# jgdumas/plinopt

Hardware: AMD Instinct MI355X
Metric: candidate SLPs/sec (higher is better)
Workload: dtype u32

## Files before the change

plinopt_amd/csrc/plo_cse_big.hip:

```cpp
#include <hip/hip_runtime.h>
#include <stdint.h>
#include <type_traits>

namespace plo {

#ifndef PLO_BIG_THREADS
#define PLO_BIG_THREADS 512
#endif
#define PLO_BIG_SELCAP 512u
#define PLO_GVB 16u
#define PLO_GVMASK 0xFFFFull
#define PLO_GEMPTY 0xFFFFFFFFFFFF0000ull

struct BigPlan {
    uint32_t m, n, nnz, p, NCmax, hbits, rb, bb, unit, maxf0, M0, multcap, dmcap, hlcap, scr_stride, aggbits, mers, agg_cb, agg_dual, selcap, prune;
    uint64_t mu;
    uint32_t nv, vt_lds;
    uint32_t mode, nr;
    const uint16_t *rtid, *invid;
    const uint32_t *rval;
    const uint32_t *rs, *ent0, *tptr, *trows, *ucount0, *hist0;
    const uint2 *vt;
    const uint32_t *invtab;
    const uint64_t *tab0;
// ... 263 lines not shown
        const uint32_t s1 = (s + 1u) & mask;
        const uint64_t v0 = __hip_atomic_load(&agg[s], __ATOMIC_RELAXED, __HIP_MEMORY_SCOPE_WORKGROUP), v1 = __hip_atomic_load(&agg[s1], __ATOMIC_RELAXED, __HIP_MEMORY_SCOPE_WORKGROUP);
        const bool hit0 = (v0 >> acb) == key, emp0 = v0 == EMPTY, first = hit0 || emp0;
        const bool hit = hit0 || (!emp0 && (v1 >> acb) == key), emp = emp0 || (!hit && v1 == EMPTY);
        const uint32_t t = first ? s : s1;
        if (hit) { wg_add((unsigned long long *)&agg[t], 1ull); done = true; break; }
        if (emp) {
            const uint64_t old = wg_cas((unsigned long long *)&agg[t], (unsigned long long)EMPTY, (unsigned long long)((key << acb) | 1ull));
            if (old == EMPTY) { claimed = t; done = true; break; }
            continue;
        }
        s = (s + 2u) & mask; pr += 2u;
    }
    const unsigned long long cm = __builtin_amdgcn_ballot_w64(claimed != 0xFFFFFFFFu);
    if (cm) {
        const uint32_t lane = threadIdx.x & 63u, leader = (uint32_t)__builtin_ctzll(cm);
        uint32_t base = 0;
        if (lane == leader) base = wg_add(aggn, (uint32_t)__builtin_popcountll(cm));
        base = (uint32_t)__builtin_amdgcn_readlane((int)base, (int)leader);
        if (claimed != 0xFFFFFFFFu) {
            const uint32_t idx = base + (uint32_t)__builtin_popcountll(cm & ((1ull << lane) - 1ull));
            if (idx < listcap) agglist[idx] = (uint16_t)claimed;
        }
    }
    return done;
}

#define PLO_RIDB 10u
#define PLO_RSTRIDE 32u
struct BigTabs { const uint2 *vts; const uint16_t *rtid; const uint32_t *rval; const uint16_t *invid; uint16_t *list; uint32_t *bloom; };
__device__ __forceinline__ bool agg_add_rid(uint32_t *aggk, uint32_t *aggc32, uint32_t aggbits, uint32_t key, uint32_t *aggn, uint16_t *agglist, uint32_t listcap) {
    const uint32_t mask = (1u << aggbits) - 1u;
    uint32_t s = (key * 0x9E3779B1u) >> (32u - aggbits);
    uint32_t claimed = 0xFFFFFFFFu; bool done = false;
    for (uint32_t pr = 0; pr < PLO_AGG_PROBES;) {
        const uint32_t s1 = (s + 1u) & mask;
        const uint32_t k0 = __hip_atomic_load(&aggk[s], __ATOMIC_RELAXED, __HIP_MEMORY_SCOPE_WORKGROUP), k1 = __hip_atomic_load(&aggk[s1], __ATOMIC_RELAXED, __HIP_MEMORY_SCOPE_WORKGROUP);
        const bool hit0 = k0 == key, emp0 = k0 == 0xFFFFFFFFu, first = hit0 || emp0;
        const bool hit = hit0 || (!emp0 && k1 == key), emp = emp0 || (!hit && k1 == 0xFFFFFFFFu);
        const uint32_t t = first ? s : s1;
        if (hit) { wg_add(&aggc32[t >> 1], 1u << ((t & 1u) << 4)); done = true; break; }
        if (emp) {
            const uint32_t old = wg_cas(&aggk[t], 0xFFFFFFFFu, key);
            if (old == 0xFFFFFFFFu || old == key) { if (old != key) claimed = t; wg_add(&aggc32[t >> 1], 1u << ((t & 1u) << 4)); done = true; break; }
            continue;
        }
        s = (s + 2u) & mask; pr += 2u;
    }
    const unsigned long long cm = __builtin_amdgcn_ballot_w64(claimed != 0xFFFFFFFFu);
    if (cm) {
        const uint32_t lane = threadIdx.x & 63u, leader = (uint32_t)__builtin_ctzll(cm);
        uint32_t base = 0;
        if (lane == leader) base = wg_add(aggn, (uint32_t)__builtin_popcountll(cm));
        base = (uint32_t)__builtin_amdgcn_readlane((int)base, (int)leader);
        if (claimed != 0xFFFFFFFFu) {
            const uint32_t idx = base + (uint32_t)__builtin_popcountll(cm & ((1ull << lane) - 1ull));
            if (idx < listcap) agglist[idx] = (uint16_t)claimed;
        }
    }
    return done;
}

__device__ __forceinline__ bool agg_add_rid_bm(uint32_t *aggk, uint32_t *aggc32, uint32_t aggbits, uint32_t key, uint32_t hshift, uint32_t *iters = nullptr) {
    const uint32_t pmask = (1u << (aggbits - 1u)) - 1u;
    uint32_t pi = (uint32_t)__umul24(key, 0x9E3779u) >> hshift;
    for (uint32_t left = PLO_AGG_PROBES / 2u;;) {
        if (iters) ++*iters;
        const unsigned long long kk = __hip_atomic_load((unsigned long long *)aggk + pi, __ATOMIC_RELAXED, __HIP_MEMORY_SCOPE_WORKGROUP);
        const uint32_t k0 = (uint32_t)kk, k1 = (uint32_t)(kk >> 32);
        const bool first = k0 == key || k0 == 0xFFFFFFFFu;
        const uint32_t kt = first ? k0 : k1;
        bool mine = kt == key;
        const uint32_t next = !mine && kt != 0xFFFFFFFFu ? 1u : 0u;
        if (kt == 0xFFFFFFFFu) {
            const uint32_t sec = first ? 0u : 1u;
            const uint32_t old = wg_cas((uint32_t *)((unsigned long long *)aggk + pi) + sec, 0xFFFFFFFFu, key);
            mine = old == 0xFFFFFFFFu || old == key;
        }
        if (mine) wg_add(&aggc32[pi], first ? 1u : 0x10000u);
        pi = (pi + next) & pmask; left -= next;
        if (mine || left == 0u) return mine;
    }
}

#ifdef PLO_BIG_PROFILE
__device__ __forceinline__ bool agg_add_rid_first_prof(uint32_t *aggk, uint32_t *aggc32, uint32_t aggbits, uint32_t key, unsigned long long *acc) {
    const unsigned long long c0 = clock64();
    const uint32_t s = ((uint32_t)__umul24(key, 0x9E3779u) >> (32u - aggbits)) & ~1u;
    const unsigned long long kk = __hip_atomic_load((unsigned long long *)(aggk + s), __ATOMIC_RELAXED, __HIP_MEMORY_SCOPE_WORKGROUP);
    const uint32_t k0 = (uint32_t)kk, k1 = (uint32_t)(kk >> 32);
    asm volatile("s_waitcnt lgkmcnt(0)" ::: "memory"); const unsigned long long c1 = clock64();
    const bool hit0 = k0 == key, hit = hit0 || k1 == key, emp0 = k0 == 0xFFFFFFFFu, tryc = !hit && (emp0 || k1 == 0xFFFFFFFFu);
    const uint32_t sec = hit ? (hit0 ? 0u : 1u) : (emp0 ? 0u : 1u), t = s + sec;
    uint32_t old = 0u;
    if (tryc) old = wg_cas(&aggk[t], 0xFFFFFFFFu, key);
    asm volatile("s_waitcnt lgkmcnt(0)" ::: "memory"); const unsigned long long c2 = clock64();
    const bool ok = hit || (tryc && (old == 0xFFFFFFFFu || old == key));
    if (ok) wg_add(&aggc32[s >> 1], sec ? 0x10000u : 1u);
    asm volatile("s_waitcnt lgkmcnt(0)" ::: "memory"); const unsigned long long c3 = clock64();
    acc[0] += c1 - c0; acc[1] += c2 - c1; acc[2] += c3 - c2;
    return !ok;
}
#endif

#define PLO_ECOL(e_) ((e_) & 0x7FFFu)
#define PLO_EUNIT(e_) (((e_) >> 15) & 1u)
#define PLO_EVI(e_) ((e_) >> 16)
#define PLO_RW_LEN 0x3FFFu
#define PLO_RW_NEW 0x1F8000u
#define PLO_RW_VIB 22u
#define PLO_RW_VIA 27u
template <class ENT> __device__ __forceinline__ int row_find(ENT ent, uint32_t base, uint32_t L, uint32_t c) {
    uint32_t lo = 0, hi = L;
    while (lo < hi) { uint32_t mid = (lo + hi) >> 1; if (PLO_ECOL(ent[base + mid]) < c) lo = mid + 1; else hi = mid; }
    return (lo < L && PLO_ECOL(ent[base + lo]) == c) ? (int)lo : -1;
}

struct BigShared {
    uint32_t M, theta, ncols, nbadd, nbmul, nmult, naff, dmcount, hlcount, rng, errflag, sel_n, sel_over, invr, fullscans, rebuilds, steps, hlbad, acc0, acc1;
    uint32_t a, b, r, aggn, nspill, keepn; uint64_t kprime; uint64_t selkey;
    uint32_t nbisect, spilltot, listover, nwin, nsearched;
    uint32_t logn, hotn, hotbits, nforced, hotops, logtot_lo, logtot_hi;
    uint32_t derr; unsigned long long tmg[4], tmb[4]; uint32_t ngrp, nloop; uint32_t outcnt[64];
    uint32_t cblk[512];
    unsigned long long tph[8];
    unsigned long long tpg[7], tld;
#ifdef PLO_BIG_PROFILE
    unsigned long long tb1[4], tb2[4]; uint32_t nb[4], fb1, fb2, fl1, fl2;
    unsigned long long tpc[4][8];
    unsigned long long pw[16];
#endif
    uint32_t part[8];
    uint64_t sel[PLO_BIG_SELCAP];
};

#define BSYNC() __syncthreads()
#ifdef PLO_BIG_PROFILE
#define PLO_STAMP(q_) do { if (threadIdx.x == 0) { unsigned long long t_ = wall_clock64(); sh.tph[q_] += t_ - tstamp; sh.tpc[sh.M >= 256u ? 0 : sh.M >= 64u ? 1 : sh.M >= 16u ? 2 : 3][q_] += t_ - tstamp; tstamp = t_; } } while (0)
#else
#define PLO_STAMP(q_) do { if (threadIdx.x == 0) { unsigned long long t_ = wall_clock64(); sh.tph[q_] += t_ - tstamp; tstamp = t_; } } while (0)
#endif

#define PLO_DLB 13u
#define PLO_DCH 4096u
#define PLO_DBIAS 0x8000u
#define PLO_DBLOOM_WORDS 4096u
#define PLO_DMREG_WORDS 16384u
#define PLO_DPMAX 2048u
#define PLO_LEMPTY (~0ull)
static_assert(PLO_DPMAX <= 4u * PLO_BIG_THREADS && PLO_DCH % PLO_BIG_THREADS == 0u && 2u * PLO_DCH + 3u * PLO_DPMAX <= PLO_DMREG_WORDS, "merge layout");

__device__ __forceinline__ uint64_t dmix(uint64_t key) { return key * 0x9E3779B97F4A7C15ull; }
__device__ __forceinline__ uint32_t dpart(uint64_t key, uint32_t pbits) { return pbits ? (uint32_t)(dmix(key) >> (64u - pbits)) : 0u; }
__device__ __forceinline__ uint32_t dlslot(uint64_t key, uint32_t pbits, uint32_t lb) { return (uint32_t)((dmix(key) << pbits) >> (64u - lb)); }
__device__ __forceinline__ bool dbloom_test(const uint32_t *bl, uint64_t key) {
    const uint64_t g = key * 0xD6E8FEB86659FD93ull;
    const uint32_t i1 = (uint32_t)(g >> 47), i2 = (uint32_t)(g >> 30) & 0x1FFFFu, i3 = (uint32_t)(g >> 13) & 0x1FFFFu;
    const uint32_t w1 = __hip_atomic_load(&bl[i1 >> 5], __ATOMIC_RELAXED, __HIP_MEMORY_SCOPE_WORKGROUP), w2 = __hip_atomic_load(&bl[i2 >> 5], __ATOMIC_RELAXED, __HIP_MEMORY_SCOPE_WORKGROUP),
                   w3 = __hip_atomic_load(&bl[i3 >> 5], __ATOMIC_RELAXED, __HIP_MEMORY_SCOPE_WORKGROUP);
    return (((w1 >> (i1 & 31u)) & (w2 >> (i2 & 31u)) & (w3 >> (i3 & 31u))) & 1u) != 0u;
}
__device__ __forceinline__ void dbloom_set(uint32_t *bl, uint64_t key) {
    const uint64_t g = key * 0xD6E8FEB86659FD93ull;
    const uint32_t i1 = (uint32_t)(g >> 47), i2 = (uint32_t)(g >> 30) & 0x1FFFFu, i3 = (uint32_t)(g >> 13) & 0x1FFFFu;
    wg_or(&bl[i1 >> 5], 1u << (i1 & 31u)); wg_or(&bl[i2 >> 5], 1u << (i2 & 31u)); wg_or(&bl[i3 >> 5], 1u << (i3 & 31u));
}
template <class TAB> __device__ __forceinline__ uint32_t hot_slot(TAB hot, uint64_t key, uint32_t hb, uint64_t &v) {
    const uint32_t mask = (1u << hb) - 1u;
    uint32_t s = ghash(key, hb);
    for (uint32_t pr = 0; pr <= mask; ++pr) {
        v = gload64(&hot[s]);
        if ((v >> PLO_GVB) == key) return s;
        if (v == PLO_GEMPTY) return 0xFFFFFFFFu;
        s = (s + 1u) & mask;
    }
    return 0xFFFFFFFFu;
}
template <class TAB> __device__ __forceinline__ uint32_t hot_addn(TAB hot, uint64_t key, uint32_t d, uint32_t hb, uint32_t *hotn) {
    const uint32_t mask = (1u << hb) - 1u;
    uint32_t s = ghash(key, hb);
    for (uint32_t pr = 0; pr <= 2u * mask + 1u; ++pr) {
        const uint64_t v = gload64(&hot[s]);
        if ((v >> PLO_GVB) == key) { const uint64_t old = wg_add((unsigned long long *)&hot[s], (unsigned long long)d); return (uint32_t)(old & PLO_GVMASK); }
        if (v == PLO_GEMPTY) {
            const uint64_t old = wg_cas((unsigned long long *)&hot[s], (unsigned long long)v, (unsigned long long)((key << PLO_GVB) | d));
            if (old == v) { wg_add(hotn, 1u); return 0u; }
// ... 496 lines not shown
        const bool swap = gload32(&ucount[a]) < gload32(&ucount[b]);
        const uint32_t l0 = swap ? b : a, l1 = swap ? a : b;
        if (tid == 0) { sh.naff = 0; sh.aggn = 0; sh.nspill = 0; sh.keepn = 0; }
        BSYNC();
#define RL(v_, k_) ((uint32_t)__builtin_amdgcn_readlane((int)(v_), (int)(k_)))
        A32 wlst; uint32_t lc;
        {
            const A32 la = a < n ? tl + tptr[a] : ncr + ncrptr[a - n], lb = b < n ? tl + tptr[b] : ncr + ncrptr[b - n];
            const uint32_t na = gload32(&clen[a]), nb = gload32(&clen[b]);
            const bool walk_a = na <= nb;
            const A32 lst = walk_a ? la : lb; const uint32_t ln = walk_a ? na : nb;
            wlst = lst; lc = walk_a ? a : b;
            if (tid == 0) sh.nsearched += ln;
            const A32 newrows = ncr + ncrptr[lm - n];
            auto emit = [&](uint32_t i, uint32_t base, uint32_t L, uint32_t pa, uint32_t pb, uint32_t ea, uint32_t eb) -> bool {
                uint32_t inv_r;
                if constexpr (MODE == 2) {
                    if (rval[rtid[PLO_EVI(eb) * PLO_RSTRIDE + PLO_EVI(ea)]] != r) return false;
                    inv_r = rval[rtid[PLO_EVI(ea) * PLO_RSTRIDE + PLO_EVI(eb)]];
                } else {
                    const uint2 A = VT(PLO_EVI(ea)), B = VT(PLO_EVI(eb));
                    if (B.x != bmul(r, A.x, p, mu, mers)) return false;
                    inv_r = bmul(A.x, B.y, p, mu, mers);
                }
                const uint32_t idx = wg_add(&sh.naff, 1u);
#ifdef PLO_BIG_PROFILE
                atomicAdd(&sh.tb2[1], 100ull * L);
#endif
                if constexpr (MODE == 2) {
                    *(uint4 *)(aff + 4u * idx) = make_uint4(pa | (pb << 16), base, L | ((swap ? eb : ea) & PLO_RW_NEW) | (PLO_EVI(eb) << PLO_RW_VIB) | (PLO_EVI(ea) << PLO_RW_VIA), i);
                } else {
                uint32_t *rec = &aff[8u * idx];
                *(uint4 *)rec = make_uint4(i, pa | (pb << 16), base, L);
                *(uint2 *)(rec + 4) = make_uint2(ea, eb);
                }
                newrows[idx] = i;
                if (idx == 0) sh.invr = inv_r;
                len[i] = L - 1u;
                if (PLO_EUNIT(ea)) wg_sub(&ucount[a], 1u);
                if (PLO_EUNIT(eb)) wg_sub(&ucount[b], 1u);
                if (PLO_EUNIT(swap ? eb : ea)) wg_add(&ucount[lm], 1u);
                return true;
            };
            auto keep_row = [&](uint32_t i, bool has_col, bool affected) { if (has_col && !affected) keep[wg_add(&sh.keepn, 1u)] = i; };
#ifdef PLO_BIG_PROFILE
            if (tid == 0) { sh.tb2[0] += 100ull * ln; sh.tb2[2] += 100ull * (na <= nb ? nb : na); }
#endif
            for (uint32_t k = tid; k < ln; k += 2u * nth) {
                const bool two = k + nth < ln;
                const uint32_t i0 = lst[k], i1 = two ? lst[k + nth] : i0;
                const uint32_t bs0 = rs[i0], bs1 = rs[i1], L0 = len[i0], L1 = two ? len[i1] : 0u;
                uint32_t lo[4] = {0u, 0u, 0u, 0u}, hi[4] = {L0, L0, L1, L1}, ev[4] = {0xFFFFFFFFu, 0xFFFFFFFFu, 0xFFFFFFFFu, 0xFFFFFFFFu};
                for (;;) {
                    uint32_t v[4], mid[4]; bool any = false;
#pragma unroll
                    for (int q = 0; q < 4; ++q) {
                        mid[q] = (lo[q] + hi[q]) >> 1; const bool go = lo[q] < hi[q]; any |= go;
                        v[q] = go ? ent[(q < 2 ? bs0 : bs1) + mid[q]] : 0u;
                    }
                    if (!any) break;
#pragma unroll
                    for (int q = 0; q < 4; ++q)
                        if (lo[q] < hi[q]) { if (PLO_ECOL(v[q]) < ((q & 1) ? b : a)) lo[q] = mid[q] + 1u; else { hi[q] = mid[q]; ev[q] = v[q]; } }
                }
                {   const bool fa = PLO_ECOL(ev[0]) == a && lo[0] < L0, fb = PLO_ECOL(ev[1]) == b && lo[1] < L0;
                    const bool aff0 = fa && fb && emit(i0, bs0, L0, lo[0], lo[1], ev[0], ev[1]);
                    keep_row(i0, walk_a ? fa : fb, aff0); }
                if (two) { const bool fa = PLO_ECOL(ev[2]) == a && lo[2] < L1, fb = PLO_ECOL(ev[3]) == b && lo[3] < L1;
                    const bool aff1 = fa && fb && emit(i1, bs1, L1, lo[2], lo[3], ev[2], ev[3]);
                    keep_row(i1, walk_a ? fa : fb, aff1); }
            }
        }
        PLO_BIG_FENCE(); BSYNC();
        const uint32_t naff = sh.naff;
        {
            const uint32_t nk = sh.keepn;
            for (uint32_t k = tid; k < nk; k += nth) wlst[k] = keep[k];
            if (tid == 0) clen[lc] = nk;
        }
        PLO_STAMP(2);
        if (naff != M) { if (tid == 0) wg_max(&sh.errflag, (uint32_t)BERR_FREQ); BSYNC(); break; }
        {
#ifdef PLO_BIG_PROFILE
            uint32_t probe_iters = 0; unsigned long long pq[3] = {0, 0, 0}, prt = 0;
#endif
            uint32_t aggsh = 33u - aggbits; asm("" : "+v"(aggsh));
            const uint32_t agg_dual = MODE == 2 ? 0u : PW(agg_dual), logcap = DEFER ? PW(logcap) : 0u;
            auto retire_entry = [&](uint32_t e, uint32_t rw, bool above, uint2 VA, uint2 VB, bool noagg = false) {
                const uint32_t c = PLO_ECOL(e);
                uint32_t x, y, q2, ins;
                if constexpr (MODE == 2) {
                    const uint32_t vi = PLO_EVI(e), via = rw >> PLO_RW_VIA;
#ifdef PLO_BIG_PROFILE
                    const unsigned long long cr0 = clock64();
#endif
                    const uint32_t xid = rtid[((above ? vi : via) * PLO_RSTRIDE) | (above ? via : vi)];
#ifdef PLO_BIG_PROFILE
                    if constexpr (FAST) {
                        asm volatile("s_waitcnt lgkmcnt(0)" ::: "memory"); prt += clock64() - cr0;
                        const bool pend = agg_add_rid_first_prof(aggk, aggc32, aggbits, (c << PLO_RIDB) | xid, pq);
                        if (!__builtin_amdgcn_ballot_w64(pend)) return;
                        if (!pend || agg_add_rid_bm(aggk, aggc32, aggbits, (c << PLO_RIDB) | xid, aggsh, &probe_iters)) return;
                    }
#else
                    if constexpr (FAST) { if (!noagg) { if (__builtin_expect(agg_add_rid_bm(aggk, aggc32, aggbits, (c << PLO_RIDB) | xid, aggsh), 1)) return; } }
#endif
                    else if (agg_add_rid(aggk, aggc32, aggbits, (c << PLO_RIDB) | xid, &sh.aggn, agglist, listcap)) return;
                    const uint32_t vib = (rw >> PLO_RW_VIB) & 31u;
                    const uint32_t bc = rval[rtid[vib * PLO_RSTRIDE + vi]];
                    x = rval[xid]; y = rval[rtid[via * PLO_RSTRIDE + vi]];
                    q2 = c < b ? bc : rval[rtid[vi * PLO_RSTRIDE + vib]];
                    ins = l0 == a ? y : bc;
                } else {
                    const uint2 V = VT(PLO_EVI(e));
                    y = bmul(VA.x, V.y, p, mu, mers);
                    x = c < a ? y : bmul(V.x, VA.y, p, mu, mers);
                    const uint64_t cx = ((uint64_t)c << rb) | x;
                    if (agg_add(agg, aggbits, acb, agg_dual ? (cx << rb) | y : cx, (uint32_t)cx ^ ((uint32_t)(cx >> 32) * 0x85EBCA6Bu), &sh.aggn, agglist, listcap)) return;
                    q2 = c < b ? bmul(VB.x, V.y, p, mu, mers) : bmul(V.x, VB.y, p, mu, mers);
                    ins = bmul(l0 == a ? VA.x : VB.x, V.y, p, mu, mers);
                }
#ifdef PLO_BIG_PROFILE
                wg_add(&sh.fb1, 1u);
#endif
                const uint64_t k1 = c < a ? BKEY(c, a, x) : BKEY(a, c, x);
                const uint64_t k2 = c < b ? BKEY(c, b, q2) : BKEY(b, c, q2);
                if constexpr (DEFER) {
                    for (int w_ = 0; w_ < 2; ++w_) {
                        const uint64_t kk = w_ ? k2 : k1; const uint32_t fc = w_ ? (c < b ? c : b) : (c < a ? c : a);
                        bool done = false;
                        if (dbloom_test(bloom, kk)) {
                            uint64_t v; const uint32_t sl = hot_slot(tab, kk, hbits, v);
                            if (sl != 0xFFFFFFFFu) {
                                const uint32_t o = (uint32_t)(wg_add((unsigned long long *)&tab[sl], ~0ull) & PLO_GVMASK);
                                if (o) { wg_sub(&hist[o], 1u); if (o > 1u) wg_add(&hist[o - 1u], 1u); if (o == M) { wg_sub(&cntM[fc], 1u); wg_sub(&sh.cblk[fc >> 6], 1u); } }
                                else wg_max(&sh.errflag, (uint32_t)BERR_TABLE);
                                done = true;
                            }
                        }
                        if (!done) { const uint32_t li = wg_add(&sh.logn, 1u); if (li < logcap) dlog[li] = PLO_DREC(kk, 1u, false); else wg_max(&sh.errflag, (uint32_t)BERR_TABLE); }
                    }
                    const uint32_t idx = wg_add(&sh.nspill, 1u);
                    if (idx < spillcap) spill[idx] = BKEY(c, lm, ins); else wg_max(&sh.errflag, (uint32_t)BERR_TABLE);
                    return;
                }
                const uint32_t o1 = gtab_dec(tab, k1, hbits);
                if (o1) {
                    wg_sub(&hist[o1], 1u); if (o1 > 1u) wg_add(&hist[o1 - 1u], 1u);
                    if (o1 == M) { wg_sub(&cntM[c < a ? c : a], 1u); wg_sub(&sh.cblk[(c < a ? c : a) >> 6], 1u); }
                }
                const uint32_t o2 = gtab_dec(tab, k2, hbits);
                if (o2) {
                    wg_sub(&hist[o2], 1u); if (o2 > 1u) wg_add(&hist[o2 - 1u], 1u);
                    if (o2 == M) { wg_sub(&cntM[c < b ? c : b], 1u); wg_sub(&sh.cblk[(c < b ? c : b) >> 6], 1u); }
                }
                const uint32_t idx = wg_add(&sh.nspill, 1u);
                if (idx < spillcap) spill[idx] = BKEY(c, lm, ins); else wg_max(&sh.errflag, (uint32_t)BERR_TABLE);
            };
            const uint32_t nrw = naff > wave ? (naff - wave + nwaves - 1u) / nwaves : 0u;
#ifdef PLO_BIG_PROFILE
            unsigned long long pw0 = 0, pw1 = 0, pw2 = 0, ptr = 0, pit = 0, pact = 0, tl_ = clock64(); const unsigned long long ts_ = tl_;
#endif
            if constexpr (FAST) {
            uint64_t *fm = sh.sel + 256u + 32u * wave;
            const uint32_t FW = PW(fwin);
            const uint32_t dump = PW(nnz) + 64u + lane;
            for (uint32_t k0 = 0; k0 < nrw; k0 += 64u) {
                const bool have = k0 + lane < nrw;
                const uint32_t qq = have ? wave + (k0 + lane) * nwaves : wave;
                const uint4 R0 = *(const uint4 *)(aff + 4u * qq);
                const uint32_t Lr = have ? (R0.z & PLO_RW_LEN) : 0u;
                const uint32_t RZ = R0.z;
                const uint32_t E = wave_incl_scan(Lr), S = E - Lr, T = RL(E, 63);
                const uint32_t safe = RL(R0.y, 0);
                uint32_t qlo = 0;
                for (uint32_t w0 = 0; w0 < T; w0 += FW) {
                    if (w0 && tid == 0) ++sh.nwin;
                    if (lane < 32u) __hip_atomic_store(&fm[lane], 0ull, __ATOMIC_RELAXED, __HIP_MEMORY_SCOPE_WORKGROUP);
                    __atomic_signal_fence(__ATOMIC_SEQ_CST); __builtin_amdgcn_wave_barrier();
                    if (have && E >= w0 && E - w0 < FW) wg_or((unsigned long long *)&fm[(E - w0) >> 6], 1ull << (E & 63u));
                    __atomic_signal_fence(__ATOMIC_SEQ_CST); __builtin_amdgcn_wave_barrier();
                    const uint64_t mreg = __hip_atomic_load(&fm[lane & 31u], __ATOMIC_RELAXED, __HIP_MEMORY_SCOPE_WORKGROUP);
                    const uint32_t mrl = (uint32_t)mreg, mrh = (uint32_t)(mreg >> 32);
                    const uint32_t ntw = ((T - w0 < FW ? T - w0 : FW) + 63u) >> 6;
                    auto prep = [&](uint32_t t_, uint32_t &ad_, uint32_t &z_, uint32_t &pp_, uint32_t &rz_, uint32_t &e_) {
                        const bool ok = t_ < ntw;
                        const uint32_t ml_ = RL(mrl, t_ & 31u), mh_ = RL(mrh, t_ & 31u);
                        const uint32_t ml = ok ? ml_ : 0u, mh = ok ? mh_ : 0u;
                        const uint32_t m1l = (ml >> 1) | (mh << 31), m1h = mh >> 1;
                        const int qa = (int)((qlo + (ml & 1u) + __builtin_amdgcn_mbcnt_hi(m1h, __builtin_amdgcn_mbcnt_lo(m1l, 0u))) << 2);
                        qlo += (uint32_t)__builtin_popcount(ml) + (uint32_t)__builtin_popcount(mh);
                        const uint32_t rb_ = (uint32_t)__builtin_amdgcn_ds_bpermute(qa, (int)R0.y), S_ = (uint32_t)__builtin_amdgcn_ds_bpermute(qa, (int)S);
                        pp_ = (uint32_t)__builtin_amdgcn_ds_bpermute(qa, (int)R0.x); rz_ = (uint32_t)__builtin_amdgcn_ds_bpermute(qa, (int)RZ);
                        const uint32_t f_ = w0 + (t_ << 6) + lane;
                        z_ = f_ - S_; ad_ = rb_ + z_;
                        e_ = ent[ok && f_ < T ? ad_ : safe];
                    };
#if !defined(PLO_BIG_PROFILE)
                    auto body3 = [&](uint32_t t, uint32_t adc, uint32_t zc, uint32_t ppc, uint32_t rzc, uint32_t ec) {
                        const uint32_t pa = ppc & 0xFFFFu, pb = ppc >> 16;
                        const bool in = w0 + (t << 6) + lane < T, act = in && zc != pa && zc != pb;
                        ent[act && zc > pa ? adc - 1u - (zc > pb ? 1u : 0u) : dump] = ec;
                        if (act) retire_entry(ec, rzc, zc > pa, make_uint2(0, 0), make_uint2(0, 0));
                    };
                    uint32_t a0_, z0_, p0_, r0_, e0_, a1_, z1_, p1_, r1_, e1_, a2_, z2_, p2_, r2_, e2_;
                    prep(0u, a0_, z0_, p0_, r0_, e0_); prep(1u, a1_, z1_, p1_, r1_, e1_);
                    __builtin_amdgcn_s_waitcnt(0x0F70);
                    for (uint32_t t = 0;;) {
                        prep(t + 2u, a2_, z2_, p2_, r2_, e2_); body3(t, a0_, z0_, p0_, r0_, e0_); if (++t >= ntw) break;
                        prep(t + 2u, a0_, z0_, p0_, r0_, e0_); body3(t, a1_, z1_, p1_, r1_, e1_); if (++t >= ntw) break;
                        prep(t + 2u, a1_, z1_, p1_, r1_, e1_); body3(t, a2_, z2_, p2_, r2_, e2_); if (++t >= ntw) break;
                    }
#else
                    uint32_t adc, zc, ppc, rzc, ec; prep(0u, adc, zc, ppc, rzc, ec);
                    __builtin_amdgcn_s_waitcnt(0x0F70);
                    for (uint32_t t = 0; t < ntw; ++t) {
                        uint32_t adn, zn, ppn, rzn, en; prep(t + 1u, adn, zn, ppn, rzn, en);
#ifdef PLO_BIG_PROFILE
                        const unsigned long long t0_ = clock64();
#endif
                        const uint32_t pa = ppc & 0xFFFFu, pb = ppc >> 16;
                        const bool in = w0 + (t << 6) + lane < T, act = in && zc != pa && zc != pb;
                        ent[act && zc > pa ? adc - 1u - (zc > pb ? 1u : 0u) : dump] = ec;
#ifdef PLO_BIG_PROFILE
                        __builtin_amdgcn_wave_barrier(); const unsigned long long t1_ = clock64(); probe_iters = 0;
#endif
                        if (act) retire_entry(ec, rzc, zc > pa, make_uint2(0, 0), make_uint2(0, 0));
#ifdef PLO_BIG_PROFILE
                        {   __builtin_amdgcn_wave_barrier(); const unsigned long long t2_ = clock64(); pw0 += t1_ - t0_; pw1 += t2_ - t1_; pw2 += t0_ - tl_; tl_ = t2_; ++ptr;
                            uint32_t mx = probe_iters; for (int o = 1; o < 64; o <<= 1) { const uint32_t u = (uint32_t)__shfl_xor((int)mx, o); mx = u > mx ? u : mx; }
                            pit += mx; pact += (unsigned long long)__builtin_popcountll(__builtin_amdgcn_ballot_w64(act)); tl_ = clock64(); }
#endif
                        adc = adn; zc = zn; ppc = ppn; rzc = rzn; ec = en;
                    }
#endif
                }
                if (have) ent[R0.y + Lr - 2u] = (R0.z & PLO_RW_NEW) | lm;
            }
            } else
            for (uint32_t k0 = 0; k0 < nrw; k0 += 64u) {
                const bool have = k0 + lane < nrw;
                const uint32_t qq = have ? wave + (k0 + lane) * nwaves : wave;
                uint32_t Rpp, Rbase, RL_, Rea, Reb;
                if constexpr (MODE == 2) {
                    const uint4 R0 = *(const uint4 *)(aff + 4u * qq);
                    Rpp = R0.x; Rbase = R0.y; RL_ = have ? (R0.z & PLO_RW_LEN) : 0u;
                    Rea = Reb = R0.z;
                } else {
                    const uint4 R0 = *(const uint4 *)(aff + 8u * qq); const uint2 R1 = *(const uint2 *)(aff + 8u * qq + 4u);
                    Rpp = R0.y; Rbase = R0.z; RL_ = have ? R0.w : 0u; Rea = R1.x; Reb = R1.y;
                }
                const uint32_t cnt = nrw - k0 < 64u ? nrw - k0 : 64u;
                uint32_t baseA = RL(Rbase, 0), LA = RL(RL_, 0), baseB = RL(Rbase, 1), LB = RL(RL_, 1);
                uint32_t eA = ent[baseA + (lane < LA ? lane : 0u)], eB = ent[baseB + (lane < LB ? lane : 0u)];
                for (uint32_t kk = 0; kk < cnt; kk += 2u) {
#ifdef PLO_BIG_PROFILE
                    unsigned long long tp = clock64();
#endif
                    const uint32_t k2 = (kk + 2u) & 63u, k3 = (kk + 3u) & 63u; const bool morep = kk + 2u < 64u;
                    const uint32_t nbaseA = RL(Rbase, k2), nLA = morep ? RL(RL_, k2) : 0u, nbaseB = RL(Rbase, k3), nLB = morep ? RL(RL_, k3) : 0u;
                    const uint32_t nfA = ent[nbaseA + (lane < nLA ? lane : 0u)], nfB = ent[nbaseB + (lane < nLB ? lane : 0u)];
                    const uint32_t ppA = RL(Rpp, kk), ppB = RL(Rpp, kk + 1u);
                    const uint32_t paA = ppA & 0xFFFFu, pbA = ppA >> 16, paB = ppB & 0xFFFFu, pbB = ppB >> 16;
                    const uint32_t eaA = RL(Rea, kk), ebA = RL(Reb, kk), eaB = RL(Rea, kk + 1u), ebB = RL(Reb, kk + 1u);
                    uint2 VaA = make_uint2(0, 0), VbA = VaA, VaB = VaA, VbB = VaA;
                    if constexpr (MODE != 2) { VaA = VT(PLO_EVI(eaA)); VbA = VT(PLO_EVI(ebA)); VaB = VT(PLO_EVI(eaB)); VbB = VT(PLO_EVI(ebB)); }
                    const uint32_t Lmax = LA > LB ? LA : LB;
                    for (uint32_t z0 = 0; z0 < Lmax; z0 += 64u) {
                        const uint32_t z = z0 + lane, zn = z + 64u;
                        const bool morez = z0 + 64u < Lmax;
                        uint32_t neA = 0, neB = 0;
                        if (morez) { neA = ent[baseA + (zn < LA ? zn : 0u)]; neB = ent[baseB + (zn < LB ? zn : 0u)]; }
                        __builtin_amdgcn_wave_barrier();
#ifdef PLO_BIG_PROFILE
                        const unsigned long long t0_ = clock64();
#endif
                        const bool actA = z < LA && z != paA && z != pbA, actB = z < LB && z != paB && z != pbB;
                        if (actA && z > paA) ent[baseA + z - 1u - (z > pbA ? 1u : 0u)] = eA;
                        if (actB && z > paB) ent[baseB + z - 1u - (z > pbB ? 1u : 0u)] = eB;
#ifdef PLO_BIG_PROFILE
                        const unsigned long long t1_ = clock64();
#endif
                        if (actA) retire_entry(eA, eaA, z > paA, VaA, VbA);
                        if (actB) retire_entry(eB, eaB, z > paB, VaB, VbB);
                        __builtin_amdgcn_wave_barrier();
#ifdef PLO_BIG_PROFILE
                        { const unsigned long long t2_ = clock64(); pw0 += t1_ - t0_; pw1 += t2_ - t1_; pw2 += t0_ - tl_; tl_ = t2_; ++ptr; }
#endif
                        if (morez) { eA = neA; eB = neB; }
                    }
                    if (lane == 0) {
                        if (LA) ent[baseA + LA - 2u] = (MODE == 2 ? eaA & PLO_RW_NEW : ((l0 == a) ? eaA : ebA) & 0xFFFF8000u) | lm;
                        if (LB) ent[baseB + LB - 2u] = (MODE == 2 ? eaB & PLO_RW_NEW : ((l0 == a) ? eaB : ebB) & 0xFFFF8000u) | lm;
                    }
                    baseA = nbaseA; LA = nLA; baseB = nbaseB; LB = nLB; eA = nfA; eB = nfB;
                }
            }
#ifdef PLO_BIG_PROFILE
            if (lane == 0 && M >= 256u) { atomicAdd(&sh.pw[0], pw0); atomicAdd(&sh.pw[1], pw1); atomicAdd(&sh.pw[2], pw2); atomicAdd(&sh.pw[3], ptr); atomicAdd(&sh.pw[4], clock64() - ts_); atomicAdd(&sh.pw[5], 1ull); atomicAdd(&sh.pw[6], pit); atomicAdd(&sh.pw[7], pact); atomicAdd(&sh.pw[8], pq[0]); atomicAdd(&sh.pw[9], pq[1]); atomicAdd(&sh.pw[10], pq[2]); atomicAdd(&sh.pw[14], prt); }
#endif
        }
#undef RL
        BSYNC();
#ifdef PLO_BIG_PROFILE
        if (tid == 0) { const int cl = M >= 256u ? 0 : M >= 64u ? 1 : M >= 16u ? 2 : 3; sh.tb1[cl] += wall_clock64() - tstamp; ++sh.nb[cl]; }
#endif
        PLO_STAMP(3);
        if constexpr (DEFER) {
            const uint32_t invr = sh.invr, theta = sh.theta;
            const uint32_t maxf0 = PW(maxf0), hlcap = PW(hlcap), dmcap = PW(dmcap), logcap = PW(logcap);
            const uint32_t agg_dual = MODE == 2 ? 0u : PW(agg_dual); const uint32_t *const invtab = MODE == 2 ? nullptr : PW(invtab);
            auto retired = [&](uint64_t k, uint32_t d, uint32_t o) {
                if (o < d) { { wg_max(&sh.errflag, (uint32_t)BERR_TABLE); wg_max(&sh.derr, 201u); } return; }
                wg_sub(&hist[o], 1u); if (o > d) wg_add(&hist[o - d], 1u);
                if (o == M) { wg_sub(&cntM[(uint32_t)(k >> abits)], 1u); wg_sub(&sh.cblk[(uint32_t)(k >> abits) >> 6], 1u); }
            };
            auto inserted = [&](uint64_t k, uint32_t o, uint32_t d) {
                const uint32_t nc = o + d;
                if (nc > maxf0 || nc > M) { wg_max(&sh.errflag, (uint32_t)BERR_FREQ); return; }
                if (o > 0u) wg_sub(&hist[o], 1u);
                wg_add(&hist[nc], 1u);
                if (o < theta && nc >= theta) { uint32_t idx = wg_add(&sh.hlcount, 1u); if (idx < hlcap) HL[idx] = k; else sh.hlbad = 1u; }
                if (nc == M) {
                    wg_add(&cntM[(uint32_t)(k >> abits)], 1u); wg_add(&sh.cblk[(uint32_t)(k >> abits) >> 6], 1u);
                    uint32_t idx = wg_add(&sh.dmcount, 1u);
                    if (idx < dmcap) DM[idx] = k; else wg_max(&sh.errflag, (uint32_t)BERR_DM);
                }
            };
            if (tid == 0) {
                uint64_t v; const uint32_t sl = hot_slot(tab, key, hbits, v);
                if (sl == 0xFFFFFFFFu || (uint32_t)(v & PLO_GVMASK) != M) { wg_max(&sh.errflag, (uint32_t)BERR_TABLE); wg_max(&sh.derr, 202u); }
                else { gstore64(&tab[sl], v - (uint64_t)M); retired(key, M, M); }
            }
            const uint32_t nent = sh.aggn, nslot = FAST ? (1u << aggbits) / 16u : nent <= listcap ? nent : (1u << aggbits);
            uint32_t nhot = 0;
            for (uint32_t s0 = 0; s0 < nslot; s0 += nth) {
              const uint32_t e_ = s0 + tid;
              uint32_t bits_ = 0;
              if constexpr (FAST) {
                  const uint32_t npair = 1u << (aggbits - 1u);
#pragma unroll
                  for (uint32_t u = 0; u < 8u; ++u) {
                      const uint32_t q = s0 * 8u + u * nth + tid; const bool in = q < npair;
                      const uint2 kq2 = ((const uint2 *)aggk)[in ? q : 0u];
                      bits_ |= in ? ((kq2.x != 0xFFFFFFFFu ? 1u : 0u) | (kq2.y != 0xFFFFFFFFu ? 2u : 0u)) << (2u * u) : 0u;
                  }
              }
              for (bool more_ = true; more_;) {
                bool valid; uint32_t s;
                if constexpr (FAST) { valid = bits_ != 0u; const uint32_t j_ = valid ? (uint32_t)__builtin_ctz(bits_) : 0u; s = valid ? 2u * (s0 * 8u + (j_ >> 1) * nth + tid) + (j_ & 1u) : 0u; bits_ &= bits_ - 1u; }
                else { valid = e_ < nslot; s = valid ? (nent <= listcap ? (uint32_t)agglist[e_] : e_) : 0u; }
                uint32_t c = 0, x = 0, y = 0, d = 0;
                if constexpr (MODE == 2) {
                    const uint32_t kq = valid ? aggk[s] : 0xFFFFFFFFu;
                    valid = kq != 0xFFFFFFFFu;
                    if (valid) {
                        d = aggc16[s]; aggk[s] = 0xFFFFFFFFu; aggc16[s] = 0; c = kq >> PLO_RIDB;
                        const uint32_t xid = kq & ((1u << PLO_RIDB) - 1u);
                        x = rval[xid]; y = rval[c > a ? (uint32_t)invid[xid] : xid];
                    }
                } else {
                    const uint64_t v = valid ? agg[s] : AEMPTY;
                    valid = v != AEMPTY;
                    if (valid) {
                        agg[s] = AEMPTY;
                        uint64_t k = v >> acb; d = (uint32_t)(v & ((1ull << acb) - 1ull));
                        if (agg_dual) { y = (uint32_t)(k & ((1ull << rb) - 1ull)); k >>= rb; }
                        c = (uint32_t)(k >> rb); x = (uint32_t)(k & ((1ull << rb) - 1ull));
                        if (!agg_dual) y = c > a ? (invtab ? invtab[x] : binv(x, p, mu, mers)) : x;
                    }
                }
                uint64_t k1 = 0, k2 = 0, k3 = 0;
                if (valid) {
                    const uint32_t ry = bmul(r, y, p, mu, mers);
                    const uint32_t x2 = c < b ? ry : bmul(x, invr, p, mu, mers);
                    k1 = c < a ? BKEY(c, a, x) : BKEY(a, c, x); k2 = c < b ? BKEY(c, b, x2) : BKEY(b, c, x2);
                    k3 = BKEY(c, lm, l0 == a ? y : ry);
                }
                bool c1 = valid, c2 = valid;
                if (valid && dbloom_test(bloom, k1)) {
                    uint64_t v; const uint32_t sl = hot_slot(tab, k1, hbits, v);
                    if (sl != 0xFFFFFFFFu) { const uint32_t o = (uint32_t)(v & PLO_GVMASK); if (o >= d) gstore64(&tab[sl], v - (uint64_t)d); retired(k1, d, o); c1 = false; ++nhot; }
// ... 635 lines not shown
```

Measured before the change: 1047.

## Process row entries in pairs per lane in the fast retire path

The fast retirement loop now has each lane handle two adjacent row entries, loaded as one 8-byte pair, instead of one. The prefix scan runs over half-lengths and the window size is halved to match. Both aggregation probes are issued before the fallback path, which only runs on failure. The software pipeline depth drops from three stages to two, and the window bitmask now uses the window-relative offset. The aim is to cut loop iterations and per-entry index and permute overhead and to add memory-level parallelism in the hash probes, at the cost of more register pressure and unaligned-pair handling for odd-length rows.

```diff
diff --git a/plinopt_amd/csrc/plo_cse_big.hip b/plinopt_amd/csrc/plo_cse_big.hip
--- a/plinopt_amd/csrc/plo_cse_big.hip
+++ b/plinopt_amd/csrc/plo_cse_big.hip
@@ -369,26 +369,6 @@
         if (mine || left == 0u) return mine;
     }
 }
-
-#ifdef PLO_BIG_PROFILE
-__device__ __forceinline__ bool agg_add_rid_first_prof(uint32_t *aggk, uint32_t *aggc32, uint32_t aggbits, uint32_t key, unsigned long long *acc) {
-    const unsigned long long c0 = clock64();
-    const uint32_t s = ((uint32_t)__umul24(key, 0x9E3779u) >> (32u - aggbits)) & ~1u;
-    const unsigned long long kk = __hip_atomic_load((unsigned long long *)(aggk + s), __ATOMIC_RELAXED, __HIP_MEMORY_SCOPE_WORKGROUP);
-    const uint32_t k0 = (uint32_t)kk, k1 = (uint32_t)(kk >> 32);
-    asm volatile("s_waitcnt lgkmcnt(0)" ::: "memory"); const unsigned long long c1 = clock64();
-    const bool hit0 = k0 == key, hit = hit0 || k1 == key, emp0 = k0 == 0xFFFFFFFFu, tryc = !hit && (emp0 || k1 == 0xFFFFFFFFu);
-    const uint32_t sec = hit ? (hit0 ? 0u : 1u) : (emp0 ? 0u : 1u), t = s + sec;
-    uint32_t old = 0u;
-    if (tryc) old = wg_cas(&aggk[t], 0xFFFFFFFFu, key);
-    asm volatile("s_waitcnt lgkmcnt(0)" ::: "memory"); const unsigned long long c2 = clock64();
-    const bool ok = hit || (tryc && (old == 0xFFFFFFFFu || old == key));
-    if (ok) wg_add(&aggc32[s >> 1], sec ? 0x10000u : 1u);
-    asm volatile("s_waitcnt lgkmcnt(0)" ::: "memory"); const unsigned long long c3 = clock64();
-    acc[0] += c1 - c0; acc[1] += c2 - c1; acc[2] += c3 - c2;
-    return !ok;
-}
-#endif
 
 #define PLO_ECOL(e_) ((e_) & 0x7FFFu)
 #define PLO_EUNIT(e_) (((e_) >> 15) & 1u)
@@ -1051,29 +1031,17 @@
         if (naff != M) { if (tid == 0) wg_max(&sh.errflag, (uint32_t)BERR_FREQ); BSYNC(); break; }
         {
 #ifdef PLO_BIG_PROFILE
-            uint32_t probe_iters = 0; unsigned long long pq[3] = {0, 0, 0}, prt = 0;
+            uint32_t probe_iters = 0; unsigned long long prt = 0;
 #endif
             uint32_t aggsh = 33u - aggbits; asm("" : "+v"(aggsh));
             const uint32_t agg_dual = MODE == 2 ? 0u : PW(agg_dual), logcap = DEFER ? PW(logcap) : 0u;
-            auto retire_entry = [&](uint32_t e, uint32_t rw, bool above, uint2 VA, uint2 VB, bool noagg = false) {
+            auto retire_entry = [&](uint32_t e, uint32_t rw, bool above, uint2 VA, uint2 VB) {
                 const uint32_t c = PLO_ECOL(e);
                 uint32_t x, y, q2, ins;
                 if constexpr (MODE == 2) {
                     const uint32_t vi = PLO_EVI(e), via = rw >> PLO_RW_VIA;
-#ifdef PLO_BIG_PROFILE
-                    const unsigned long long cr0 = clock64();
-#endif
                     const uint32_t xid = rtid[((above ? vi : via) * PLO_RSTRIDE) | (above ? via : vi)];
-#ifdef PLO_BIG_PROFILE
-                    if constexpr (FAST) {
-                        asm volatile("s_waitcnt lgkmcnt(0)" ::: "memory"); prt += clock64() - cr0;
-                        const bool pend = agg_add_rid_first_prof(aggk, aggc32, aggbits, (c << PLO_RIDB) | xid, pq);
-                        if (!__builtin_amdgcn_ballot_w64(pend)) return;
-                        if (!pend || agg_add_rid_bm(aggk, aggc32, aggbits, (c << PLO_RIDB) | xid, aggsh, &probe_iters)) return;
-                    }
-#else
-                    if constexpr (FAST) { if (!noagg) { if (__builtin_expect(agg_add_rid_bm(aggk, aggc32, aggbits, (c << PLO_RIDB) | xid, aggsh), 1)) return; } }
-#endif
+                    if constexpr (FAST) { }
                     else if (agg_add_rid(aggk, aggc32, aggbits, (c << PLO_RIDB) | xid, &sh.aggn, agglist, listcap)) return;
                     const uint32_t vib = (rw >> PLO_RW_VIB) & 31u;
                     const uint32_t bc = rval[rtid[vib * PLO_RSTRIDE + vi]];
@@ -1126,13 +1094,40 @@
                 const uint32_t idx = wg_add(&sh.nspill, 1u);
                 if (idx < spillcap) spill[idx] = BKEY(c, lm, ins); else wg_max(&sh.errflag, (uint32_t)BERR_TABLE);
             };
+            auto retire_pair = [&](uint32_t e0, uint32_t e1, bool act0, bool act1, uint32_t rw, bool above0, bool above1) {
+                if constexpr (FAST) {
+                    const uint32_t via = rw >> PLO_RW_VIA, vi0 = PLO_EVI(e0), vi1 = PLO_EVI(e1);
+#ifdef PLO_BIG_PROFILE
+                    const unsigned long long cr0 = clock64();
+#endif
+                    const uint32_t xid0 = rtid[((above0 ? vi0 : via) * PLO_RSTRIDE) | (above0 ? via : vi0)];
+                    const uint32_t xid1 = rtid[((above1 ? vi1 : via) * PLO_RSTRIDE) | (above1 ? via : vi1)];
+#ifdef PLO_BIG_PROFILE
+                    asm volatile("s_waitcnt lgkmcnt(0)" ::: "memory"); prt += clock64() - cr0;
+#endif
+                    const uint32_t key0 = (PLO_ECOL(e0) << PLO_RIDB) | xid0, key1 = (PLO_ECOL(e1) << PLO_RIDB) | xid1;
+#ifdef PLO_BIG_PROFILE
+                    uint32_t *const it_ = &probe_iters;
+#else
+                    uint32_t *const it_ = nullptr;
+#endif
+                    uint32_t fail = 0u;
+                    if (act0 && !agg_add_rid_bm(aggk, aggc32, aggbits, key0, aggsh, it_)) fail |= 1u;
+                    if (act1 && !agg_add_rid_bm(aggk, aggc32, aggbits, key1, aggsh, it_)) fail |= 2u;
+                    if (__builtin_expect(fail != 0u, 0)) {
+                        if (fail & 1u) retire_entry(e0, rw, above0, make_uint2(0, 0), make_uint2(0, 0));
+                        if (fail & 2u) retire_entry(e1, rw, above1, make_uint2(0, 0), make_uint2(0, 0));
+                    }
+                }
+            };
             const uint32_t nrw = naff > wave ? (naff - wave + nwaves - 1u) / nwaves : 0u;
 #ifdef PLO_BIG_PROFILE
             unsigned long long pw0 = 0, pw1 = 0, pw2 = 0, ptr = 0, pit = 0, pact = 0, tl_ = clock64(); const unsigned long long ts_ = tl_;
 #endif
             if constexpr (FAST) {
+            struct __attribute__((packed, aligned(4))) EntPair { uint32_t x, y; };
             uint64_t *fm = sh.sel + 256u + 32u * wave;
-            const uint32_t FW = PW(fwin);
+            const uint32_t FW = PW(fwin) >> 1;
             const uint32_t dump = PW(nnz) + 64u + lane;
             for (uint32_t k0 = 0; k0 < nrw; k0 += 64u) {
                 const bool have = k0 + lane < nrw;
@@ -1140,19 +1135,20 @@
                 const uint4 R0 = *(const uint4 *)(aff + 4u * qq);
                 const uint32_t Lr = have ? (R0.z & PLO_RW_LEN) : 0u;
                 const uint32_t RZ = R0.z;
-                const uint32_t E = wave_incl_scan(Lr), S = E - Lr, T = RL(E, 63);
+                const uint32_t Lp = (Lr + 1u) >> 1;
+                const uint32_t E = wave_incl_scan(Lp), S = E - Lp, T = RL(E, 63);
                 const uint32_t safe = RL(R0.y, 0);
                 uint32_t qlo = 0;
                 for (uint32_t w0 = 0; w0 < T; w0 += FW) {
                     if (w0 && tid == 0) ++sh.nwin;
                     if (lane < 32u) __hip_atomic_store(&fm[lane], 0ull, __ATOMIC_RELAXED, __HIP_MEMORY_SCOPE_WORKGROUP);
                     __atomic_signal_fence(__ATOMIC_SEQ_CST); __builtin_amdgcn_wave_barrier();
-                    if (have && E >= w0 && E - w0 < FW) wg_or((unsigned long long *)&fm[(E - w0) >> 6], 1ull << (E & 63u));
+                    if (have && E >= w0 && E - w0 < FW) wg_or((unsigned long long *)&fm[(E - w0) >> 6], 1ull << ((E - w0) & 63u));
                     __atomic_signal_fence(__ATOMIC_SEQ_CST); __builtin_amdgcn_wave_barrier();
                     const uint64_t mreg = __hip_atomic_load(&fm[lane & 31u], __ATOMIC_RELAXED, __HIP_MEMORY_SCOPE_WORKGROUP);
                     const uint32_t mrl = (uint32_t)mreg, mrh = (uint32_t)(mreg >> 32);
-                    const uint32_t ntw = ((T - w0 < FW ? T - w0 : FW) + 63u) >> 6;
-                    auto prep = [&](uint32_t t_, uint32_t &ad_, uint32_t &z_, uint32_t &pp_, uint32_t &rz_, uint32_t &e_) {
+                    const uint32_t Tw = T - w0 < FW ? T : w0 + FW, ntw = (Tw - w0 + 63u) >> 6;
+                    auto prep = [&](uint32_t t_, uint32_t &ad_, uint32_t &z_, uint32_t &pp_, uint32_t &rz_, EntPair &e_) {
                         const bool ok = t_ < ntw;
                         const uint32_t ml_ = RL(mrl, t_ & 31u), mh_ = RL(mrh, t_ & 31u);
                         const uint32_t ml = ok ? ml_ : 0u, mh = ok ? mh_ : 0u;
@@ -1162,47 +1158,35 @@
                         const uint32_t rb_ = (uint32_t)__builtin_amdgcn_ds_bpermute(qa, (int)R0.y), S_ = (uint32_t)__builtin_amdgcn_ds_bpermute(qa, (int)S);
                         pp_ = (uint32_t)__builtin_amdgcn_ds_bpermute(qa, (int)R0.x); rz_ = (uint32_t)__builtin_amdgcn_ds_bpermute(qa, (int)RZ);
                         const uint32_t f_ = w0 + (t_ << 6) + lane;
-                        z_ = f_ - S_; ad_ = rb_ + z_;
-                        e_ = ent[ok && f_ < T ? ad_ : safe];
+                        z_ = (f_ - S_) << 1; ad_ = rb_ + z_;
+                        e_ = *(const EntPair *)&ent[f_ < Tw ? ad_ : safe];
                     };
-#if !defined(PLO_BIG_PROFILE)
-                    auto body3 = [&](uint32_t t, uint32_t adc, uint32_t zc, uint32_t ppc, uint32_t rzc, uint32_t ec) {
-                        const uint32_t pa = ppc & 0xFFFFu, pb = ppc >> 16;
-                        const bool in = w0 + (t << 6) + lane < T, act = in && zc != pa && zc != pb;
-                        ent[act && zc > pa ? adc - 1u - (zc > pb ? 1u : 0u) : dump] = ec;
-                        if (act) retire_entry(ec, rzc, zc > pa, make_uint2(0, 0), make_uint2(0, 0));
+                    auto body = [&](uint32_t t, uint32_t adc, uint32_t zc, uint32_t ppc, uint32_t rzc, EntPair ec) {
+#ifdef PLO_BIG_PROFILE
+                        const unsigned long long t0_ = clock64();
+#endif
+                        const uint32_t pa = ppc & 0xFFFFu, pb = ppc >> 16, z1 = zc + 1u;
+                        const bool in = w0 + (t << 6) + lane < Tw;
+                        const bool act0 = in && zc != pa && zc != pb, act1 = in && z1 < (rzc & PLO_RW_LEN) && z1 != pa && z1 != pb;
+                        ent[act0 && zc > pa ? adc - 1u - (zc > pb ? 1u : 0u) : dump] = ec.x;
+                        ent[act1 && z1 > pa ? adc - (z1 > pb ? 1u : 0u) : dump] = ec.y;
+#ifdef PLO_BIG_PROFILE
+                        __builtin_amdgcn_wave_barrier(); const unsigned long long t1_ = clock64(); probe_iters = 0;
+#endif
+                        if (act0 || act1) retire_pair(ec.x, ec.y, act0, act1, rzc, zc > pa, z1 > pa);
+#ifdef PLO_BIG_PROFILE
+                        {   __builtin_amdgcn_wave_barrier(); const unsigned long long t2_ = clock64(); pw0 += t1_ - t0_; pw1 += t2_ - t1_; pw2 += t0_ - tl_; tl_ = t2_; ++ptr;
+                            uint32_t mx = probe_iters; for (int o = 1; o < 64; o <<= 1) { const uint32_t u = (uint32_t)__shfl_xor((int)mx, o); mx = u > mx ? u : mx; }
+                            pit += mx; pact += (unsigned long long)(__builtin_popcountll(__builtin_amdgcn_ballot_w64(act0)) + __builtin_popcountll(__builtin_amdgcn_ballot_w64(act1))); tl_ = clock64(); }
+#endif
                     };
-                    uint32_t a0_, z0_, p0_, r0_, e0_, a1_, z1_, p1_, r1_, e1_, a2_, z2_, p2_, r2_, e2_;
-                    prep(0u, a0_, z0_, p0_, r0_, e0_); prep(1u, a1_, z1_, p1_, r1_, e1_);
+                    uint32_t a0_, z0_, p0_, r0_, a1_, z1_, p1_, r1_; EntPair e0_, e1_;
+                    prep(0u, a0_, z0_, p0_, r0_, e0_);
                     __builtin_amdgcn_s_waitcnt(0x0F70);
                     for (uint32_t t = 0;;) {
-                        prep(t + 2u, a2_, z2_, p2_, r2_, e2_); body3(t, a0_, z0_, p0_, r0_, e0_); if (++t >= ntw) break;
-                        prep(t + 2u, a0_, z0_, p0_, r0_, e0_); body3(t, a1_, z1_, p1_, r1_, e1_); if (++t >= ntw) break;
-                        prep(t + 2u, a1_, z1_, p1_, r1_, e1_); body3(t, a2_, z2_, p2_, r2_, e2_); if (++t >= ntw) break;
+                        prep(t + 1u, a1_, z1_, p1_, r1_, e1_); body(t, a0_, z0_, p0_, r0_, e0_); if (++t >= ntw) break;
+                        prep(t + 1u, a0_, z0_, p0_, r0_, e0_); body(t, a1_, z1_, p1_, r1_, e1_); if (++t >= ntw) break;
                     }
-#else
-                    uint32_t adc, zc, ppc, rzc, ec; prep(0u, adc, zc, ppc, rzc, ec);
-                    __builtin_amdgcn_s_waitcnt(0x0F70);
-                    for (uint32_t t = 0; t < ntw; ++t) {
-                        uint32_t adn, zn, ppn, rzn, en; prep(t + 1u, adn, zn, ppn, rzn, en);
-#ifdef PLO_BIG_PROFILE
-                        const unsigned long long t0_ = clock64();
-#endif
-                        const uint32_t pa = ppc & 0xFFFFu, pb = ppc >> 16;
-                        const bool in = w0 + (t << 6) + lane < T, act = in && zc != pa && zc != pb;
-                        ent[act && zc > pa ? adc - 1u - (zc > pb ? 1u : 0u) : dump] = ec;
-#ifdef PLO_BIG_PROFILE
-                        __builtin_amdgcn_wave_barrier(); const unsigned long long t1_ = clock64(); probe_iters = 0;
-#endif
-                        if (act) retire_entry(ec, rzc, zc > pa, make_uint2(0, 0), make_uint2(0, 0));
-#ifdef PLO_BIG_PROFILE
-                        {   __builtin_amdgcn_wave_barrier(); const unsigned long long t2_ = clock64(); pw0 += t1_ - t0_; pw1 += t2_ - t1_; pw2 += t0_ - tl_; tl_ = t2_; ++ptr;
-                            uint32_t mx = probe_iters; for (int o = 1; o < 64; o <<= 1) { const uint32_t u = (uint32_t)__shfl_xor((int)mx, o); mx = u > mx ? u : mx; }
-                            pit += mx; pact += (unsigned long long)__builtin_popcountll(__builtin_amdgcn_ballot_w64(act)); tl_ = clock64(); }
-#endif
-                        adc = adn; zc = zn; ppc = ppn; rzc = rzn; ec = en;
-                    }
-#endif
                 }
                 if (have) ent[R0.y + Lr - 2u] = (R0.z & PLO_RW_NEW) | lm;
             }
@@ -1266,7 +1250,7 @@
                 }
             }
 #ifdef PLO_BIG_PROFILE
-            if (lane == 0 && M >= 256u) { atomicAdd(&sh.pw[0], pw0); atomicAdd(&sh.pw[1], pw1); atomicAdd(&sh.pw[2], pw2); atomicAdd(&sh.pw[3], ptr); atomicAdd(&sh.pw[4], clock64() - ts_); atomicAdd(&sh.pw[5], 1ull); atomicAdd(&sh.pw[6], pit); atomicAdd(&sh.pw[7], pact); atomicAdd(&sh.pw[8], pq[0]); atomicAdd(&sh.pw[9], pq[1]); atomicAdd(&sh.pw[10], pq[2]); atomicAdd(&sh.pw[14], prt); }
+            if (lane == 0 && M >= 256u) { atomicAdd(&sh.pw[0], pw0); atomicAdd(&sh.pw[1], pw1); atomicAdd(&sh.pw[2], pw2); atomicAdd(&sh.pw[3], ptr); atomicAdd(&sh.pw[4], clock64() - ts_); atomicAdd(&sh.pw[5], 1ull); atomicAdd(&sh.pw[6], pit); atomicAdd(&sh.pw[7], pact); atomicAdd(&sh.pw[14], prt); }
 #endif
         }
 #undef RL
```

Result: faster. 1087 (median of 6 runs) (+3.8%).
